# motroy/orion-kmer

Measured on AMD Instinct MI355X. Metric: bases/sec k-mer-counted (k=31) at 1/2/4/8 MI355X; achieved HBM GB/s vs peak, higher is better.
Workload: dtype u64

## Files before the change

orion-kmer_amd/csrc/okm_count.hip:

```cpp
#include "okm_dev_common.h"

namespace okm {

constexpr int kCountWpe = 8;
constexpr int kFullHomeBitsW = 12;

constexpr int kCB = 512;
constexpr int kPer = 8;
constexpr int kCapI = kCB * kPer;
constexpr int kHomeBits = kCB == 512 ? 11 : 10;
constexpr int kHomes = 1 << kHomeBits;
constexpr int kHomesPer = kHomes / kCB;
constexpr int kDenseBits = kHomeBits;
constexpr int kLoadU = 4;

constexpr int kTagBytes = kHomes * 8;
constexpr int kPairBytes = kHomes * 2;
template <bool W> struct Lds {
    static constexpr int kTcntBytes = W ? kHomes * 8 : kPairBytes;
    static constexpr int kRc = kTagBytes + kTcntBytes;
    static constexpr int kHd = kRc + kPairBytes;
    static constexpr int kLt = kHd + kPairBytes;
    static constexpr int kFixed = kLt + kPairBytes;
    static constexpr int kRestEntry = W ? 17 : 9;
// ... 5 lines not shown
    static_assert(kHomes * 12 <= kBytes, "dense mode must fit the carve-up");
};

uint32_t count_item_capacity() { return kCapI; }
uint32_t count_dense_bits() { return kDenseBits; }

template <bool W>
struct CountType {
    typedef uint32_t T;
};
template <>
struct CountType<true> {
    typedef ull T;
};

__device__ __forceinline__ uint32_t wave_incl_scan32(uint32_t v) {
    const int lane = threadIdx.x & 63;
#pragma unroll
    for (int d = 1; d < 64; d <<= 1) {
        const uint32_t o = __shfl_up(v, d, 64);
        if (lane >= d) v += o;
    }
    return v;
}

__device__ __forceinline__ void lds_only_sync();
template <bool LDS_ONLY = false>
__device__ __forceinline__ uint32_t block_excl_scan32(uint32_t v, uint32_t *wsum, uint32_t *total) {
    const int lane = threadIdx.x & 63, wid = threadIdx.x >> 6;
    const uint32_t inc = wave_incl_scan32(v);
    if (lane == 63) wsum[wid] = inc;
    if (LDS_ONLY) lds_only_sync(); else lds_sync();
    uint32_t wbase = 0, tot = 0;
#pragma unroll
    for (int w = 0; w < kCB / 64; ++w) {
        const uint32_t s = wsum[w];
        wbase += w < wid ? s : 0u;
        tot += s;
    }
    if (LDS_ONLY) lds_only_sync(); else lds_sync();
// ... 86 lines not shown
    uint32_t sbase = 0;
    for (uint32_t sg = 0; sg < it.seg_count; ++sg) {
        const DevSeg s = segs[it.seg_begin + sg];
        const uint32_t len = (uint32_t)s.len;
#pragma unroll
        for (int u = 0; u < kPer; ++u) {
            if ((uint32_t)u * kCB >= sbase + len) break;
            const uint32_t f = (uint32_t)u * kCB + t - sbase;
            if (f < len) {
                kk[u] = gload(reinterpret_cast<const KT *>(s.keys) + f);
                if (W && s.counts) ww[u] = gload(s.counts + f);
            }
        }
        sbase += len;
    }
}

constexpr int kSegCache = 64;
template <bool W, typename KT = ull>
__device__ __forceinline__ void load_item_segs(const DevItem &it, const DevSeg *__restrict__ segs, KT (&kk)[kPer],
                                               ull (&ww)[kPer], const uint64_t **ck, const uint64_t **cc,
                                               uint32_t *coff) {
    const uint32_t t = threadIdx.x;
    const uint32_t R = __builtin_amdgcn_readfirstlane(it.seg_count);
    lds_sync();
    if (t < R) {
        const DevSeg s = segs[it.seg_begin + t];
        ck[t] = s.keys;
        cc[t] = s.counts;
        coff[t + 1] = (uint32_t)s.len;
// ... 276 lines not shown
        okeys[p] = sk[b];
        ull c = 0;
        if (W)
            for (uint32_t i = b; i < e; ++i) c += sw[i];
        else
            c = e - b;
        store_count<W>(out_counts, out_off + p, c, narrow, ctl);
    }
    return __builtin_amdgcn_readfirstlane(D);
}


constexpr uint32_t kDeferred = ~0u;

template <bool W, bool NW = false>
__device__ __forceinline__ uint32_t tag_item(const DevItem &it, const DevSeg *__restrict__ segs, uint32_t nrows,
                                             const ull (&kk)[kPer], const ull (&ww)[kPer], ull *lds, uint32_t *wsum,
                                             uint64_t *__restrict__ out_keys, uint64_t *__restrict__ out_counts,
                                             bool narrow, ull *ctl) {
    const uint32_t r = it.rem_bits;
    const uint64_t out_off = it.out_off;
    ull *okeys = out_slot_keys<ull>(it, out_keys);
    typedef Lds<W> L;
    typedef typename CountType<W>::T CT;
    const uint32_t t = threadIdx.x;
    char *base = reinterpret_cast<char *>(lds);
    ull *tag = lds;
    uint32_t *tc16 = reinterpret_cast<uint32_t *>(lds + kHomes);
    ull *tc64 = lds + kHomes;
    uint32_t *rc = reinterpret_cast<uint32_t *>(base + L::kRc);
    uint32_t *hd = reinterpret_cast<uint32_t *>(base + L::kHd);
    uint32_t *lt = reinterpret_cast<uint32_t *>(base + L::kLt);
    ull *rk = reinterpret_cast<ull *>(base + L::kFixed);
    ull *rw = rk + L::kRest;
    uint8_t *rf = reinterpret_cast<uint8_t *>(rk + (W ? 2 : 1) * L::kRest);

    uint32_t hp[kPer];
#pragma unroll
    for (int u = 0; u < kPer; ++u) {
        if ((uint32_t)u >= nrows) break;
        hp[u] = ~0u;
        const ull x = kk[u];
        if (x != kEmptyKey) {
            const uint32_t h = home_of(x, r);
            const ull old = atomicCAS(&tag[h], kEmptyKey, x);
            if (old == kEmptyKey || old == x) {
                if (W)
                    atomicAdd(&tc64[h], ww[u]);
                else
                    atomicAdd(&tc16[h >> 1], 1u << half_shift(h));
            } else {
                const uint32_t o = atomicAdd(&rc[h >> 1], 1u << half_shift(h));
                hp[u] = (h << 16) | half_of(o, h);
            }
        }
    }
    lds_sync();
    hd[2 * t] = hd[2 * t + 1] = 0;
    {
        const uint32_t w0 = rc[2 * t], w1 = rc[2 * t + 1];
        const uint32_t c0 = w0 & 0xFFFFu, c1 = w0 >> 16, c2 = w1 & 0xFFFFu;
        uint32_t rtot;
        const uint32_t a = block_excl_scan32(c0 + c1 + c2 + (w1 >> 16), wsum, &rtot);
// ... 1 lines not shown
            tag_reset<W>(lds);
            return kDeferred;
        }
        rc[2 * t] = a | ((a + c0) << 16);
        rc[2 * t + 1] = (a + c0 + c1) | ((a + c0 + c1 + c2) << 16);
        if (t == 0) wsum[kCB / 64] = rtot;
    }
    lds_sync();
#pragma unroll
    for (int u = 0; u < kPer; ++u) {
        if ((uint32_t)u >= nrows) break;
        if (hp[u] != ~0u) {
            const uint32_t h = hp[u] >> 16;
            const uint32_t dst = half_of(rc[h >> 1], h) + (hp[u] & 0xFFFFu);
            rk[dst] = kk[u];
            if (W) rw[dst] = ww[u];
        }
    }
    lds_sync();
    const uint32_t rtot = __builtin_amdgcn_readfirstlane(wsum[kCB / 64]);
    ull px[L::kRestIters];
    CT pc[L::kRestIters];
    uint32_t prange[L::kRestIters];
#pragma unroll
    for (int k = 0; k < L::kRestIters; ++k) {
        prange[k] = 0;
        if ((uint32_t)k * kCB >= rtot) break;
        const uint32_t p = (uint32_t)k * kCB + t;
        if (p < rtot) {
            const ull x = rk[p];
            const uint32_t h = home_of(x, r);
// ... 44 lines not shown
#pragma unroll
        for (int q = 0; q < kHomesPer; ++q) {
            tg[q] = tag[kHomesPer * t + q];
            tag[kHomesPer * t + q] = kEmptyKey;
            dq[q] += tg[q] != kEmptyKey;
            ho[q] = d;
            d += dq[q];
        }
        const uint32_t od = block_excl_scan32(d, wsum, &D);
#pragma unroll
        for (int q = 0; q < kHomesPer; ++q) ho[q] += od;
        hd[2 * t] = ho[0] | (ho[1] << 16);
        hd[2 * t + 1] = ho[2] | (ho[3] << 16);
    }
    lds_sync();
    {
        const uint32_t lq[kHomesPer] = {lw0 & 0xFFFFu, lw0 >> 16, lw1 & 0xFFFFu, lw1 >> 16};
        uint32_t nq[kHomesPer];
        if (!W) {
            nq[0] = nw0 & 0xFFFFu;
            nq[1] = nw0 >> 16;
            nq[2] = nw1 & 0xFFFFu;
            nq[3] = nw1 >> 16;
        }
#pragma unroll
        for (int q = 0; q < kHomesPer; ++q) {
            if (!NW && tg[q] != kEmptyKey) {
                const uint64_t o = out_off + ho[q] + lq[q];
                okeys[o - out_off] = tg[q];
                const uint64_t cq = W ? (uint64_t)tw[q] : (uint64_t)nq[q];
                store_count<W>(out_counts, o, cq, narrow, ctl);
            }
        }
    }
#pragma unroll
    for (int k = 0; k < L::kRestIters; ++k) {
        if (NW || (uint32_t)k * kCB >= rtot) break;
        if (prange[k]) {
            const ull x = px[k];
            const uint32_t hs = (prange[k] >> 16) & 0x7FFFu, he = prange[k] & 0xFFFFu;
            uint32_t less = 0;
            for (uint32_t q = hs; q < he; ++q) less += (rf[q] && rk[q] < x) ? 1u : 0u;
            const uint32_t h = home_of(x, r);
            const uint32_t tag_below = prange[k] >> 31;
            const uint64_t o = out_off + half_of(hd[h >> 1], h) + less + tag_below;
            okeys[o - out_off] = x;
            store_count<W>(out_counts, o, (uint64_t)pc[k], narrow, ctl);
        }
    }
    return __builtin_amdgcn_readfirstlane(D);
}


template <bool W, typename KT>
__device__ __forceinline__ uint32_t dense_item(const DevItem &it, const DevSeg *__restrict__ segs,
                                               uint64_t *__restrict__ out_keys_raw, uint64_t *__restrict__ out_counts,
                                               ull *lds, uint32_t *wsum, bool nowrite, bool narrow, ull *ctl,
                                               const Direct *dir = nullptr) {
    typedef typename CountType<W>::T CT;
    const uint32_t t = threadIdx.x;
    const uint32_t r = it.rem_bits;
    const uint32_t nslots = 1u << r;
// ... 46 lines not shown
            }
        }
        return __builtin_amdgcn_readfirstlane(D);
    }
    for (uint32_t q = 0; q < kHomesPer; ++q) {
        const uint32_t j = t * kHomesPer + q;
        if (!nowrite && j < nslots && cnt[j] != 0) {
            okeys[o - it.out_off] = slot_key[j];
            store_count<W>(out_counts, o, (uint64_t)cnt[j], narrow, ctl);
            ++o;
        }
    }
    return __builtin_amdgcn_readfirstlane(D);
}

template <bool W, bool NW = false, bool NARROW = !W>
__global__ __launch_bounds__(kCB) __attribute__((amdgpu_waves_per_eu(W ? 1 : kCountWpe)))
void k_count_items(const DevItem *__restrict__ items, uint32_t nitems, const DevSeg *__restrict__ segs,
                   uint64_t *__restrict__ out_keys, uint64_t *__restrict__ out_counts, ull *__restrict__ n_out,
                   ull *__restrict__ ctl, uint32_t *__restrict__ defer, const ull *__restrict__ guard,
                   const ull *__restrict__ d_nitems) {
    if (guard && (guard[0] | guard[1])) return;
    if (d_nitems) nitems = __builtin_amdgcn_readfirstlane((uint32_t)min((ull)nitems, *d_nitems));
    __shared__ __attribute__((aligned(16))) ull lds[Lds<W>::kBytes / 8];
    __shared__ uint32_t wsum[kCB / 64 + 1];
    const uint64_t **seg_k = reinterpret_cast<const uint64_t **>(reinterpret_cast<char *>(lds) + Lds<W>::kFixed);
    const uint64_t **seg_c = seg_k + kSegCache;
    uint32_t *seg_off = reinterpret_cast<uint32_t *>(seg_c + kSegCache);
    static_assert(kSegCache * 20 + 4 <= Lds<W>::kRest * 8, "segment cache fits the rest buffer");
    const uint32_t t = threadIdx.x;
    tag_reset<W>(lds);
    for (uint32_t item = blockIdx.x; item < nitems; item += gridDim.x) {
        const DevItem it = items[item];
        const uint64_t total = it.pad == kItemEmpty ? 0 : item_total(it, segs);
        if (total == 0) {
            if (t == 0) n_out[item] = 0;
            continue;
        }
        uint32_t written = kDeferred;
        if (it.rem_bits > (uint32_t)kDenseBits && total <= (uint64_t)kCapI) {
            ull kk[kPer];
            ull ww[kPer];
            if (W && it.seg_count > 1 && it.seg_count <= (uint32_t)kSegCache)
                load_item_segs<W>(it, segs, kk, ww, seg_k, seg_c, seg_off);
            else
                load_item<W>(it, segs, kk, ww);
            const uint32_t nrows = (uint32_t)((total + kCB - 1) / kCB);
            written = tag_item<W, NW>(it, segs, nrows, kk, ww, lds, wsum, out_keys, out_counts, NARROW, ctl);
        }
        if (t == 0) {
            if (written == kDeferred)
                defer[atomicAdd(reinterpret_cast<unsigned int *>(ctl + 1), 1u)] = item;
            else
                n_out[item] = written;
        }
    }
}

template <typename KT, bool W, bool DIRECT = false>
__global__ __launch_bounds__(kCB) __attribute__((amdgpu_waves_per_eu((W && sizeof(KT) > 8) ? 1 : 4))) void k_count_slow(const DevItem *__restrict__ items, uint32_t nitems,
                                                    const DevSeg *__restrict__ segs,
                                                    uint64_t *__restrict__ out_keys,
                                                    uint64_t *__restrict__ out_counts, ull *__restrict__ n_out,
// ... 52 lines not shown
            written = full_item<W, KT, kHB, DIRECT>(it, (uint32_t)((total + kCB - 1) / kCB), kk, ww, lds, wsum,
                                                    out_keys, out_counts, nowrite, narrow, ctl, dir);
        } else {
            if (threadIdx.x == 0) atomicOr(reinterpret_cast<unsigned int *>(ctl), 2u);
            if (DIRECT) (void)lookback(dsc, 0, ctl);
        }
        if (threadIdx.x == 0) n_out[item] = written;
        lds_sync();
    }
}

void launch_count_items(void *stream, const DevItem *items, uint32_t nitems, const DevSeg *segs,
                        uint64_t *out_keys, uint64_t *out_counts, unsigned long long *n_out,
                        unsigned long long *ctl, uint32_t *defer, bool weighted, bool wide,
                        const unsigned long long *guard, const unsigned long long *d_nitems, bool nowrite,
                        bool narrow) {
    if (!nitems) return;
    hipStream_t s = (hipStream_t)stream;
    constexpr uint32_t wide_cap = 8191, weighted_cap = 4095;
    if (wide) {
        const uint32_t grid = nitems < wide_cap ? nitems : wide_cap;
        if (weighted)
            hipLaunchKernelGGL((k_count_slow<K128, true>), dim3(grid), dim3(kCB), 0, s, items, nitems, segs, out_keys,
                               out_counts, n_out, ctl, (const uint32_t *)nullptr, guard, d_nitems, nowrite, narrow,
                               (ull *)nullptr, (uint64_t *)nullptr, (uint64_t *)nullptr, (const ull *)nullptr);
        else
            hipLaunchKernelGGL((k_count_slow<K128, false>), dim3(grid), dim3(kCB), 0, s, items, nitems, segs,
                               out_keys, out_counts, n_out, ctl, (const uint32_t *)nullptr, guard, d_nitems, nowrite,
                               narrow, (ull *)nullptr, (uint64_t *)nullptr, (uint64_t *)nullptr, (const ull *)nullptr);
        return;
    }
// ... 3 lines not shown
    const uint32_t sgrid = nitems < 1023u ? nitems : 1023u;
    if (weighted) {
        if (nowrite)
            hipLaunchKernelGGL((k_count_items<true, true>), dim3(wgrid), dim3(kCB), 0, s, items, nitems, segs,
                               out_keys, out_counts, n_out, ctl, defer, guard, d_nitems);
        else if (narrow)
            hipLaunchKernelGGL((k_count_items<true, false, true>), dim3(wgrid), dim3(kCB), 0, s, items, nitems, segs,
                               out_keys, out_counts, n_out, ctl, defer, guard, d_nitems);
        else
            hipLaunchKernelGGL((k_count_items<true, false, false>), dim3(wgrid), dim3(kCB), 0, s, items, nitems,
                               segs, out_keys, out_counts, n_out, ctl, defer, guard, d_nitems);
        hipLaunchKernelGGL((k_count_slow<ull, true>), dim3(sgrid), dim3(kCB), 0, s, items, nitems, segs, out_keys,
                           out_counts, n_out, ctl, (const uint32_t *)defer, guard, d_nitems, nowrite, narrow,
                           (ull *)nullptr, (uint64_t *)nullptr, (uint64_t *)nullptr, (const ull *)nullptr);
    } else {
        hipLaunchKernelGGL(k_count_items<false>, dim3(grid), dim3(kCB), 0, s, items, nitems, segs, out_keys,
                           out_counts, n_out, ctl, defer, guard, d_nitems);
        hipLaunchKernelGGL((k_count_slow<ull, false>), dim3(sgrid), dim3(kCB), 0, s, items, nitems, segs, out_keys,
                           out_counts, n_out, ctl, (const uint32_t *)defer, guard, d_nitems, nowrite, narrow,
                           (ull *)nullptr, (uint64_t *)nullptr, (uint64_t *)nullptr, (const ull *)nullptr);
    }
}

void launch_count_direct(void *stream, const DevItem *items, uint32_t nitems, const DevSeg *segs,
                         unsigned long long *n_out, unsigned long long *ctl, bool weighted,
                         const unsigned long long *guard, const unsigned long long *d_nitems,
                         unsigned long long *status, uint64_t *fin_keys, uint64_t *fin_counts,
                         const unsigned long long *fin_base) {
    if (!nitems) return;
    hipStream_t s = (hipStream_t)stream;
    const uint32_t grid = nitems < 2048u ? nitems : 2048u;
    if (weighted)
// ... 11 lines not shown
```

orion-kmer_amd/csrc/okm_dev_common.h:

```cpp
#pragma once

#include <hip/hip_runtime.h>

#include "okm_internal.h"
#include "okm_key.h"

namespace okm {

typedef unsigned long long ull;

__device__ __forceinline__ void lds_sync() { __syncthreads(); }

template <typename T>
__device__ __forceinline__ T gload(const T *p) {
    return *(const __attribute__((address_space(1))) T *)p;
}
__device__ __forceinline__ K128 gload(const K128 *p) {
    typedef unsigned long long u64x2 __attribute__((ext_vector_type(2)));
    const u64x2 v = *(const __attribute__((address_space(1))) u64x2 *)p;
    return K128{v.x, v.y};
}
__device__ __forceinline__ uint4 gload(const uint4 *p) {
    typedef unsigned int u32x4 __attribute__((ext_vector_type(4)));
    const u32x4 v = *(const __attribute__((address_space(1))) u32x4 *)p;
// ... 33 lines not shown
    const int lane = threadIdx.x & 63, wid = threadIdx.x >> 6;
    const ull inc = wave_incl_scan(v);
    if (lane == 63) wsum[wid] = inc;
    lds_sync();
    ull wbase = 0, tot = 0;
#pragma unroll
    for (int w = 0; w < BLOCK / 64; ++w) {
        const ull s = wsum[w];
        if (w < wid) wbase += s;
        tot += s;
    }
    *total = tot;
    return wbase + inc - v;
}

}
```

orion-kmer_amd/csrc/okm_engine.hip:

```cpp
#include <hip/hip_runtime.h>

#include <algorithm>
#include <cmath>
#include <chrono>
#include <cstdio>
#include <cstdlib>
#include <cstring>
#include <map>
#include <memory>
#include <atomic>
#include <mutex>
#include <string>
#include <vector>

#include "okm_arena.h"
#include "okm_hip_try.h"
#include "okm_internal.h"
#include "okm_key.h"
#include "orion_kmer_testing.h"

namespace okm {

static thread_local std::string g_last_error;

// ... 1316 lines not shown
    return OKM_OK;
}

struct ResDst {
    uint64_t *keys, *counts;
    uint64_t off;
    unsigned long long *d_base = nullptr;
    unsigned long long *hslot = nullptr;
};

static okm_status count_and_compact(okm_ctx *c, DevItem *d_items, DevSeg *d_segs, uint32_t nitems,
                                    uint64_t out_total, uint64_t in_total, bool weighted, Blocks &level,
                                    Blocks &items, const unsigned long long *guard = nullptr,
                                    unsigned long long *hguard = nullptr, bool *aborted = nullptr,
                                    const unsigned long long *d_nitems = nullptr, const ResDst *dst = nullptr,
                                    bool last_use = false, bool in_place = false) {
    uint64_t *sk = nullptr, *sc = nullptr;
    unsigned long long *n_out, *dense_off, *scan_tmp;
    const bool direct = dst && c->wide;
    bool narrow = !direct && (!weighted || (!in_place && !dst));
    const uint64_t sc_words = narrow ? (std::max<uint64_t>(out_total, 1) + 1) / 2 : std::max<uint64_t>(out_total, 1);
    if (last_use && c->may_take_runs && !dst && !in_place) {
        const size_t need = std::max<uint64_t>(out_total, 1) * 8 * c->kw;
        size_t best = 0;
        for (auto &r : c->runs) {
            const size_t b = r.borrowed ? 0 : c->pool->size_of(r.keys);
            if (b >= need && (!best || b < best)) best = b, sk = r.keys;
        }
    }
    const bool donated = sk != nullptr;
    Lost lost{c};
// ... 23 lines not shown
                c->pool->size_of(sc) / 1e9, (sk && !donated ? c->pool->size_of(sk) : 0) / 1e9);
    }
    HIP_TRY(hipMemsetAsync(c->flag, 0, 2 * sizeof(unsigned long long), c->stream));
    HIP_TRY(hipMemsetAsync(d_nitems ? n_out : n_out + nitems, 0,
                           (d_nitems ? nitems + 1 : 1) * sizeof(unsigned long long), c->stream));
    if (direct) HIP_TRY(hipMemsetAsync(status, 0, (size_t)nitems * sizeof(unsigned long long), c->stream));
    c->timer.begin(c->stream);
    c->hprof.mark("items.h2d");
    lost.on = donated;
    if (direct)
        launch_count_direct(c->stream, d_items, nitems, d_segs, n_out, c->flag, weighted, guard, d_nitems, status,
                            dst->d_base ? dst->keys : dst->keys + dst->off * c->kw,
                            dst->d_base ? dst->counts : dst->counts + dst->off, dst->d_base);
    else
        launch_count_items(c->stream, d_items, nitems, d_segs, sk, sc, n_out, c->flag, defer, weighted, c->wide, guard,
                           d_nitems, false, narrow);
    c->timer.end(c->stream, "count_items", (8.0 * c->kw + (weighted ? 8.0 : 0.0)) * (double)in_total);
    HIP_TRY(hipGetLastError());
    launch_exclusive_scan(c->stream, n_out, dense_off, nitems + 1, scan_tmp);
    HIP_TRY(hipGetLastError());
    if (dst && !direct) {
        c->timer.begin(c->stream);
        if (dst->d_base)
            launch_compact_items(c->stream, d_items, nitems, n_out, dense_off, sk, sc, dst->keys, dst->counts, c->wide,
                                 !weighted, guard, c->flag, d_nitems, dst->d_base);
        else
            launch_compact_items(c->stream, d_items, nitems, n_out, dense_off, sk, sc, dst->keys + dst->off * c->kw,
                                 dst->counts + dst->off, c->wide, !weighted, guard, c->flag, d_nitems);
        c->timer.end(c->stream, "compact_items", 0.0);
        HIP_TRY(hipGetLastError());
    }
// ... 33 lines not shown
            lost.on = false;
            own.free_all();
            return OKM_OK;
        }
    }
    if (weighted && narrow && hv[1] == 8) {
        c->hprof.mark("count.narrow_overflow");
        own.put(sc);
        sc = nullptr;
        narrow = false;
        OKM_TRY(own.get(std::max<uint64_t>(out_total, 1), &sc));
        HIP_TRY(hipMemsetAsync(c->flag, 0, 2 * sizeof(unsigned long long), c->stream));
        HIP_TRY(hipMemsetAsync(d_nitems ? n_out : n_out + nitems, 0,
                               (d_nitems ? nitems + 1 : 1) * sizeof(unsigned long long), c->stream));
        launch_count_items(c->stream, d_items, nitems, d_segs, sk, sc, n_out, c->flag, defer, weighted, c->wide, guard,
                           d_nitems, false, false);
        HIP_TRY(hipGetLastError());
        launch_exclusive_scan(c->stream, n_out, dense_off, nitems + 1, scan_tmp);
        HIP_TRY(hipMemcpyAsync(&hv[0], dense_off + nitems, sizeof(unsigned long long), hipMemcpyDeviceToHost, c->stream));
        HIP_TRY(hipMemcpyAsync(&hv[1], c->flag, sizeof(unsigned long long), hipMemcpyDeviceToHost, c->stream));
        OKM_TRY(sync(c));
    }
    if (hv[1]) return fail(OKM_E_DEVICE, "count_items invariant violated (code " + std::to_string(hv[1]) + ")");
    const uint64_t nd = hv[0];
    const uint32_t nkept = d_nitems ? (uint32_t)std::min<unsigned long long>(nitems, hv[5]) : nitems;
    const double staged = 8.0 * c->kw + (narrow ? 4.0 : 8.0);
    const double dense = 8.0 * c->kw + 8.0;
    if (!c->timer.stats.empty()) {
        c->timer.stats[c->timer.id_of("count_items")].alg_bytes += (direct ? dense : staged) * (double)nd;
        if (dst && !direct) c->timer.add_bytes("compact_items", (staged + dense) * (double)nd);
    }
// ... 339 lines not shown
                        (unsigned long long)r.n, r.sorted, r.folded, r.borrowed,
                        (unsigned long long)(r.off.empty() ? 0 : r.off.back()));
        }
        bufs.free_all();
        items.free_all();
        *fallback = true;
        return OKM_OK;
    }
    c->info.max_partition = hf[1];
    const int64_t mkv = test_knob(OKM_TEST_SORTED_PATH);
    const double need = 2.0 * (8.0 * c->kw + 8.0) * (double)in_total;
    const bool tight = need > 0.9 * device_room(c);
    const bool two_pass = weighted && (mkv == 2 || (tight && mkv != 1));
    const bool merge = (mkv == 1 || tight) && R <= merge_max_runs() && item_max <= merge_item_capacity();
    if (!two_pass && !merge)
        return count_and_compact(c, d_items, d_segs, nitems, in_total, in_total, weighted, bufs, items);
    items.move_to(bufs);
    if (two_pass) return count_sorted_two_pass(c, d_items, d_segs, nitems, in_total, bufs);
    return merge_sorted_items(c, d_items, d_segs, nitems, in_total, weighted, bufs);
}

struct CountPlan {
    uint32_t twok;
    uint64_t item_max;
    uint32_t capbits;
    uint64_t target;
    uint32_t maxb;
};
static okm_status count_parts(okm_ctx *c, std::vector<DevSeg> &segtab, std::vector<Part> &parts, bool weighted,
                              const CountPlan &cp, const ResDst *dst);
static okm_status count_grouped(okm_ctx *c, std::vector<DevSeg> &segtab, std::vector<Part> &parts, bool weighted,
// ... 427 lines not shown
    }
    c->info.work_items = nitems;
    if (nitems == 0) {
        level.free_all();
        c->counted = true;
        c->n_res = 0;
        c->info.distinct = 0;
        return OKM_OK;
    }
    OKM_TRY(items.get(segtab.size(), &d_segs));
    OKM_TRY(items.get(nitems, &d_items));
    OKM_TRY(h2d(c, d_segs, segtab.data(), segtab.size() * sizeof(DevSeg)));
    OKM_TRY(h2d(c, d_items, host_items.data(), nitems * sizeof(DevItem)));
    c->hprof.mark("items.build");
    return count_and_compact(c, d_items, d_segs, nitems, out_total, in_total, weighted, level, items, nullptr, nullptr,
                             nullptr, nullptr, dst, false, one_seg && !level.held().empty());
}

static okm_status count_grouped(okm_ctx *c, std::vector<DevSeg> &segtab, std::vector<Part> &parts, bool weighted,
                                const CountPlan &cp) {
    uint64_t total = 0;
    for (const Part &p : parts) total += p.len;
    const double ws_key = 8.0 * c->kw * 3 + (weighted ? 8.0 : 4.0) + (weighted ? 16.0 : 0.0);
    const double res_key = 8.0 * c->kw + 8.0;
    const double one_key = std::max(ws_key, 8.0 * c->kw + (weighted ? 8.0 : 4.0) + res_key);
    const double room = device_room(c);
    const double avail = 0.75 * room;
    uint64_t group_keys = total;
    int mode = 0;
    bool over_ok = false;
    if (!weighted && c->may_take_runs && c->runs.size() == 1) {
// ... 823 lines not shown
```

orion-kmer_amd/csrc/okm_extract.hip:

```cpp
#include "okm_scan.h"

namespace okm {

__device__ __forceinline__ uint32_t bin_of(uint64_t key, uint32_t shift) {
    return shift >= 64 ? 0u : (uint32_t)(key >> shift);
}
template <int K>
__device__ __forceinline__ uint32_t bin_k(uint64_t key, uint32_t shift) {
    if (K >= 21) return (uint32_t)(key >> 32) >> (shift - 32u);
    return bin_of(key, shift);
}

constexpr int kExtractBlock = 256;
constexpr int kScatBlock = 1024;
constexpr int kScatWpe = 4;
constexpr int kSegS = 16;
constexpr int kTile = kScatBlock * kSegS;
static_assert(kSegS % 16 == 0, "scan_windows loads whole 16-B words");
constexpr int kSegH = 64;
constexpr int kHTile = kExtractBlock * kSegH;
static_assert(kHTile % kTile == 0, "scatter tile must divide the hist tile");
constexpr int kL1Bits = 9, kL1BitsFold = 10, kL1BitsW = 9;
constexpr int kMaxL1Bins = 1 << kL1BitsFold;
static_assert(2 * 21 - kL1BitsFold >= 32, "bin_k: the L1 shift of k >= 21 lies in the key's high word");
// ... 56 lines not shown
            else
                atomicOr(ovf, 1ull);
        }
        gcur[t] = g;
    }
}

template <int K>
__global__ __launch_bounds__(kScatBlock) __attribute__((amdgpu_waves_per_eu(kScatWpe))) void k_extract_scatter(
    const uint8_t *__restrict__ seq, ExtractGeom g, const uint32_t *__restrict__ HC, ull *__restrict__ cursor,
    uint64_t *__restrict__ out, const ull *__restrict__ cap_end, ull *__restrict__ ovf) {
    __shared__ ull stage[kTile + 64];
    __shared__ ull gcur[kMaxL1Bins];
    __shared__ uint32_t hist[kMaxL1Bins + 1];
    __shared__ uint32_t lofs[kMaxL1Bins];
    __shared__ ull wsum[kScatBlock / 64];
    const uint32_t t = threadIdx.x;
    const uint32_t nb = g.nbins;
    if (t < nb && HC) {
        const uint32_t h = HC[(uint64_t)blockIdx.x * nb + t];
        gcur[t] = h ? atomicAdd(&cursor[t], (ull)h) : 0ull;
    }
    const uint64_t beg = (uint64_t)blockIdx.x * g.chunk;
    const uint64_t end = beg + g.chunk < g.n ? beg + g.chunk : g.n;
    const uint32_t shift = g.shift;
    WinWords<kSegS> ww;
    load_windows_clamped<kSegS>(seq, g.n, beg + (uint64_t)t * kSegS, ww);
    const ull capb = (!HC && t < nb) ? cap_end[t] : 0ull;
    for (uint32_t b = t; b <= nb; b += kScatBlock) hist[b] = 0;
    lds_sync();
    for (uint64_t t0 = beg; t0 < end; t0 += kTile) {
// ... 7 lines not shown
            uint32_t vm = 0;
#pragma unroll
            for (int j = 0; j < kSegS / 2; ++j) rk[j] = 0;
            auto emit = [&](int j, uint64_t key, bool valid) {
                const uint32_t b = valid ? bin_k<K>(key, shift) : nb;
                kk[j] = key;
                rk[j >> 1] |= (atomicAdd(&hist[b], 1u) & 0xFFFFu) << (16 * (j & 1));
                vm |= valid ? 1u << j : 0u;
            };
            if (live) scan_words<kSegS, K>(ww, g.k, emit, g.n - w0);
            load_windows_clamped<kSegS>(seq, g.n, w0 + kTile, ww);
            lds_sync();
            hmine = t <= nb ? hist[t] : 0u;
            if (t <= nb) hist[t] = 0;
            {
                ull tn;
                const uint32_t off = (uint32_t)block_excl_scan_1b<kScatBlock>(t < nb ? hmine : 0u, wsum, &tn);
                if (t < nb) lofs[t] = off;
                tile_n = (uint32_t)tn;
            }
            uint32_t ch = 0;
            ull cp;
            if (!HC && t < nb) {
                ch = hmine;
                cp = atomicAdd(&cursor[t * kL1CurStride], (ull)ch);
            }
            lds_sync();
#pragma unroll
            for (int j = 0; j < kSegS; ++j) {
                const uint32_t rank = (rk[j >> 1] >> (16 * (j & 1))) & 0xFFFFu;
                const uint32_t dst = (vm >> j) & 1u ? lofs[bin_k<K>(kk[j], shift)] + rank : (uint32_t)kTile + (t & 63u);
                stage[dst] = kk[j];
            }
            if (!HC && t < nb) {
// ... 288 lines not shown
```

orion-kmer_amd/csrc/okm_internal.h:

```cpp
#pragma once

#include <stdint.h>
#include <stddef.h>
#include <string>
#include <vector>

#include "orion_kmer.h"

namespace okm {

void set_error(const std::string &msg);
okm_status fail(okm_status s, const std::string &msg);

constexpr uint64_t kEmptyKey = ~0ull;

void *host_pinned_alloc(size_t bytes);
void host_pinned_free(void *p);
okm_status memcpy_d2h_on(int device, void *dst, const void *src, size_t bytes);
int64_t test_knob(int knob);
bool test_fail_alloc();

void trim_device_pools(int device);
void device_bytes_add(int device, int64_t delta);
bool device_over_budget(int device, size_t bytes);
// ... 80 lines not shown
uint32_t extract_max_bins(bool wide);
uint32_t extract_l1_bits(bool wide, bool folding);
uint32_t part_max_bins(bool weighted, bool wide);

size_t scan_tmp_elems(uint64_t n);
void launch_exclusive_scan(void *stream, const unsigned long long *in, unsigned long long *out,
                           uint64_t n, unsigned long long *tmp);

uint32_t count_item_capacity();
uint32_t count_dense_bits();
void launch_count_items(void *stream, const DevItem *items, uint32_t nitems, const DevSeg *segs,
                        uint64_t *out_keys, uint64_t *out_counts, unsigned long long *n_out,
                        unsigned long long *ctl, uint32_t *defer, bool weighted, bool wide,
                        const unsigned long long *guard = nullptr, const unsigned long long *d_nitems = nullptr,
                        bool nowrite = false,
                        bool narrow = false);
void launch_count_direct(void *stream, const DevItem *items, uint32_t nitems, const DevSeg *segs,
                         unsigned long long *n_out, unsigned long long *ctl, bool weighted,
                         const unsigned long long *guard, const unsigned long long *d_nitems,
                         unsigned long long *status, uint64_t *fin_keys, uint64_t *fin_counts,
                         const unsigned long long *fin_base);

uint32_t merge_item_capacity();
uint32_t merge_max_runs();
void launch_merge_items(void *stream, const DevItem *items, uint32_t nitems, const DevSeg *segs,
                        unsigned long long *n_out, const unsigned long long *dense_off, uint64_t *out_keys,
                        uint64_t *out_counts, unsigned long long *ctl, bool weighted, bool wide, bool write);

struct DevParent {
    uint32_t out_base;
    uint32_t rem;
// ... 67 lines not shown
```

orion-kmer_amd/csrc/okm_partition.hip:

```cpp
#include "okm_dev_common.h"

namespace okm {

constexpr int kPartBlock = 1024;
constexpr int kHistU = 4;

uint32_t part_max_bins(bool weighted, bool wide) {
    return weighted ? 512u : (!wide ? 2u * kPartBlock : (uint32_t)kPartBlock);
}

template <typename KT>
__device__ __forceinline__ uint32_t local_bin(const KT &key, const DevSeg &s) {
    const uint64_t b = (s.shift >= (uint32_t)KeyOps<KT>::kBits ? 0ull : KeyOps<KT>::shr(key, s.shift)) - s.key_base;
    return b < s.nlocal ? (uint32_t)b : s.nlocal - 1;
}

template <typename KT>
__device__ __forceinline__ void hist_key(const KT &key, const DevSeg &s, uint32_t *lh) {
    if (!KeyOps<KT>::is_empty(key)) atomicAdd(&lh[local_bin(key, s)], 1u);
}

template <typename KT>
__global__ __launch_bounds__(kPartBlock) void k_part_hist(const DevSeg *__restrict__ segs,
                                                          const DevChunk *__restrict__ chunks,
// ... 56 lines not shown
template <typename KT, bool W, bool BIG = false>
__global__ __launch_bounds__(kPartBlock) __attribute__((amdgpu_waves_per_eu(1)))
void k_part_scatter_tile(
    const DevSeg *__restrict__ segs, const DevChunk *__restrict__ chunks, uint32_t nchunks,
    uint32_t max_local, const uint32_t *__restrict__ HC, ull *__restrict__ cursor,
    uint64_t *__restrict__ out_keys_raw, uint64_t *__restrict__ out_counts, const ull *__restrict__ cap_end,
    ull *__restrict__ ovf) {
    constexpr int T = Tile<KT, W, BIG>::kKeys, P = Tile<KT, W, BIG>::kPer;
    constexpr uint32_t BPT = BIG ? 2 : 1;
    extern __shared__ __attribute__((aligned(16))) ull lds[];
    KT *stage = reinterpret_cast<KT *>(lds);
    ull *cstage = reinterpret_cast<ull *>(stage + T);
    ull *gcur = W ? cstage + T : cstage;
    uint32_t *hist = reinterpret_cast<uint32_t *>(gcur + max_local);
    uint32_t *lofs = hist + max_local;
    __shared__ ull wsum[kPartBlock / 64];
    KT *out_keys = reinterpret_cast<KT *>(out_keys_raw);
    const uint32_t t = threadIdx.x;

    for (uint32_t c = blockIdx.x; c < nchunks; c += gridDim.x) {
        const DevChunk ch = chunks[c];
        const DevSeg s = segs[ch.seg];
        const uint32_t nl = s.nlocal;
        if (HC)
            for (uint32_t b = t; b < nl; b += kPartBlock) {
                const uint32_t h = HC[(uint64_t)c * max_local + b];
                gcur[b] = h ? atomicAdd(&cursor[s.out_base + b], (ull)h) : 0ull;
            }
        const KT *keys = reinterpret_cast<const KT *>(s.keys) + ch.begin;
        const uint64_t *cnts = s.counts ? s.counts + ch.begin : nullptr;
        for (uint64_t base = 0; base < ch.len; base += T) {
// ... 19 lines not shown
            lds_sync();
            uint32_t my[BPT];
            uint32_t mine = 0;
#pragma unroll
            for (uint32_t q = 0; q < BPT; ++q) {
                const uint32_t b = BPT * t + q;
                my[q] = b < nl ? hist[b] : 0u;
                mine += my[q];
            }
            ull claim[BPT];
#pragma unroll
            for (uint32_t q = 0; q < BPT; ++q) {
                claim[q] = 0;
                if (!HC && my[q]) claim[q] = atomicAdd(&cursor[s.out_base + BPT * t + q], (ull)my[q]);
            }
            ull tile_n;
            uint32_t off = (uint32_t)block_excl_scan<kPartBlock>(mine, wsum, &tile_n);
#pragma unroll
            for (uint32_t q = 0; q < BPT; ++q) {
                if (BPT * t + q < nl) lofs[BPT * t + q] = off;
                off += my[q];
            }
            lds_sync();
#pragma unroll
            for (int u = 0; u < P; ++u) {
                if (br[u] != ~0u) {
                    const uint32_t dst = lofs[br[u] >> 16] + (br[u] & 0xFFFFu);
                    stage[dst] = kk[u];
                    if (W) cstage[dst] = ww[u];
                }
            }
            if (!HC) {
#pragma unroll
                for (uint32_t q = 0; q < BPT; ++q) {
                    const uint32_t b = BPT * t + q;
                    if (b >= nl) continue;
                    ull g = ~0ull;
                    if (my[q]) {
                        if (claim[q] + my[q] <= cap_end[s.out_base + b])
                            g = claim[q];
                        else
                            atomicOr(ovf, 1ull);
                    }
                    gcur[b] = g;
                }
            }
            lds_sync();
            for (uint32_t j = t; j < (uint32_t)tile_n; j += kPartBlock) {
                const KT key = stage[j];
                const uint32_t b = local_bin(key, s);
                const ull g = gcur[b];
                if (g == ~0ull) continue;
                const ull o = g + (j - lofs[b]);
                out_keys[o] = key;
                if (W) out_counts[o] = cstage[j];
            }
            lds_sync();
            if (HC)
                for (uint32_t b = t; b < nl; b += kPartBlock) gcur[b] += hist[b];
        }
        lds_sync();
    }
}
// ... 70 lines not shown
```

Measured before the change: 113.3 billion.

## Add single-segment count kernel, DPP wave scan, and 32-bit block scans

Adds a specialized unweighted count-items kernel for the single-segment case. It loads keys directly from keys0 without the segment loop and reads item fields through a pointer instead of copying the whole struct. The shuffle-based wave scan is replaced with DPP row operations. Partition and extract now use a 32-bit block scan in place of the 64-bit one, and output stores go through address-space-1 pointer arithmetic with 32-bit indices. These changes aim to cut instruction count, register use and cross-lane overhead, at the cost of another template variant and new correctness assumptions, such as indices fitting in 32 bits and the item layout.

After: 121.7 billion, median of 6. 1.07x the previous value.

```diff
diff --git a/orion-kmer_amd/csrc/okm_count.hip b/orion-kmer_amd/csrc/okm_count.hip
--- a/orion-kmer_amd/csrc/okm_count.hip
+++ b/orion-kmer_amd/csrc/okm_count.hip
@@ -43,16 +43,6 @@
     typedef ull T;
 };
 
-__device__ __forceinline__ uint32_t wave_incl_scan32(uint32_t v) {
-    const int lane = threadIdx.x & 63;
-#pragma unroll
-    for (int d = 1; d < 64; d <<= 1) {
-        const uint32_t o = __shfl_up(v, d, 64);
-        if (lane >= d) v += o;
-    }
-    return v;
-}
-
 __device__ __forceinline__ void lds_only_sync();
 template <bool LDS_ONLY = false>
 __device__ __forceinline__ uint32_t block_excl_scan32(uint32_t v, uint32_t *wsum, uint32_t *total) {
@@ -169,6 +159,22 @@
         }
         sbase += len;
     }
+}
+
+__device__ __forceinline__ void load_item_one(const uint64_t *__restrict__ keys, uint32_t len, ull (&kk)[kPer]) {
+    const uint32_t t = threadIdx.x;
+#pragma unroll
+    for (int u = 0; u < kPer; ++u) {
+        const uint32_t f = (uint32_t)u * kCB + t;
+        kk[u] = kEmptyKey;
+        if (f < len) kk[u] = gload(reinterpret_cast<const ull *>(keys) + f);
+    }
+}
+
+typedef __attribute__((address_space(1))) char gchar;
+template <typename T>
+__device__ __forceinline__ void gstore_at(gchar *base, uint32_t idx, T v) {
+    *reinterpret_cast<__attribute__((address_space(1))) T *>(base + idx * (uint32_t)sizeof(T)) = v;
 }
 
 constexpr int kSegCache = 64;
@@ -475,13 +481,10 @@
 constexpr uint32_t kDeferred = ~0u;
 
 template <bool W, bool NW = false>
-__device__ __forceinline__ uint32_t tag_item(const DevItem &it, const DevSeg *__restrict__ segs, uint32_t nrows,
-                                             const ull (&kk)[kPer], const ull (&ww)[kPer], ull *lds, uint32_t *wsum,
-                                             uint64_t *__restrict__ out_keys, uint64_t *__restrict__ out_counts,
-                                             bool narrow, ull *ctl) {
-    const uint32_t r = it.rem_bits;
-    const uint64_t out_off = it.out_off;
-    ull *okeys = out_slot_keys<ull>(it, out_keys);
+__device__ __forceinline__ uint32_t tag_item(const DevItem *__restrict__ ip, uint32_t r, uint32_t nrows,
+                                             const ull (&kk)[kPer], const ull (&ww)[W ? kPer : 1], ull *lds,
+                                             uint32_t *wsum, uint64_t *__restrict__ out_keys,
+                                             uint64_t *__restrict__ out_counts, bool narrow, ull *ctl) {
     typedef Lds<W> L;
     typedef typename CountType<W>::T CT;
     const uint32_t t = threadIdx.x;
@@ -498,16 +501,17 @@
 
     uint32_t hp[kPer];
 #pragma unroll
+    for (int u = 0; u < kPer; ++u) hp[u] = ~0u;
+#pragma unroll
     for (int u = 0; u < kPer; ++u) {
         if ((uint32_t)u >= nrows) break;
-        hp[u] = ~0u;
         const ull x = kk[u];
         if (x != kEmptyKey) {
             const uint32_t h = home_of(x, r);
             const ull old = atomicCAS(&tag[h], kEmptyKey, x);
             if (old == kEmptyKey || old == x) {
                 if (W)
-                    atomicAdd(&tc64[h], ww[u]);
+                    atomicAdd(&tc64[h], ww[W ? u : 0]);
                 else
                     atomicAdd(&tc16[h >> 1], 1u << half_shift(h));
             } else {
@@ -539,7 +543,7 @@
             const uint32_t h = hp[u] >> 16;
             const uint32_t dst = half_of(rc[h >> 1], h) + (hp[u] & 0xFFFFu);
             rk[dst] = kk[u];
-            if (W) rw[dst] = ww[u];
+            if (W) rw[dst] = ww[W ? u : 0];
         }
     }
     lds_sync();
@@ -614,6 +618,20 @@
         hd[2 * t + 1] = ho[2] | (ho[3] << 16);
     }
     lds_sync();
+    if (NW) return __builtin_amdgcn_readfirstlane(D);
+    const uint64_t out_off = ip->out_off;
+    gchar *const okeys = out_keys ? (gchar *)(out_keys + out_off) : (gchar *)ip->keys0;
+    const bool c64 = W && !narrow;
+    gchar *const ocnt = (gchar *)out_counts + out_off * (c64 ? 8u : 4u);
+    auto put = [&](uint32_t o, ull key, uint64_t c) {
+        gstore_at<ull>(okeys, o, key);
+        if (c64) {
+            gstore_at<ull>(ocnt, o, c);
+        } else {
+            if (W && c > 0xFFFFFFFFull) atomicOr(reinterpret_cast<unsigned int *>(ctl), 8u);
+            gstore_at<uint32_t>(ocnt, o, (uint32_t)c);
+        }
+    };
     {
         const uint32_t lq[kHomesPer] = {lw0 & 0xFFFFu, lw0 >> 16, lw1 & 0xFFFFu, lw1 >> 16};
         uint32_t nq[kHomesPer];
@@ -625,17 +643,12 @@
         }
 #pragma unroll
         for (int q = 0; q < kHomesPer; ++q) {
-            if (!NW && tg[q] != kEmptyKey) {
-                const uint64_t o = out_off + ho[q] + lq[q];
-                okeys[o - out_off] = tg[q];
-                const uint64_t cq = W ? (uint64_t)tw[q] : (uint64_t)nq[q];
-                store_count<W>(out_counts, o, cq, narrow, ctl);
-            }
+            if (tg[q] != kEmptyKey) put(ho[q] + lq[q], tg[q], W ? (uint64_t)tw[W ? q : 0] : (uint64_t)nq[q]);
         }
     }
 #pragma unroll
     for (int k = 0; k < L::kRestIters; ++k) {
-        if (NW || (uint32_t)k * kCB >= rtot) break;
+        if ((uint32_t)k * kCB >= rtot) break;
         if (prange[k]) {
             const ull x = px[k];
             const uint32_t hs = (prange[k] >> 16) & 0x7FFFu, he = prange[k] & 0xFFFFu;
@@ -643,9 +656,7 @@
             for (uint32_t q = hs; q < he; ++q) less += (rf[q] && rk[q] < x) ? 1u : 0u;
             const uint32_t h = home_of(x, r);
             const uint32_t tag_below = prange[k] >> 31;
-            const uint64_t o = out_off + half_of(hd[h >> 1], h) + less + tag_below;
-            okeys[o - out_off] = x;
-            store_count<W>(out_counts, o, (uint64_t)pc[k], narrow, ctl);
+            put(half_of(hd[h >> 1], h) + less + tag_below, x, (uint64_t)pc[k]);
         }
     }
     return __builtin_amdgcn_readfirstlane(D);
@@ -722,7 +733,7 @@
     return __builtin_amdgcn_readfirstlane(D);
 }
 
-template <bool W, bool NW = false, bool NARROW = !W>
+template <bool W, bool NW = false, bool NARROW = !W, bool SEG1 = false>
 __global__ __launch_bounds__(kCB) __attribute__((amdgpu_waves_per_eu(W ? 1 : kCountWpe)))
 void k_count_items(const DevItem *__restrict__ items, uint32_t nitems, const DevSeg *__restrict__ segs,
                    uint64_t *__restrict__ out_keys, uint64_t *__restrict__ out_counts, ull *__restrict__ n_out,
@@ -738,8 +749,34 @@
     static_assert(kSegCache * 20 + 4 <= Lds<W>::kRest * 8, "segment cache fits the rest buffer");
     const uint32_t t = threadIdx.x;
     tag_reset<W>(lds);
+    static_assert(!(SEG1 && W), "the single-segment kernel is the unweighted one");
     for (uint32_t item = blockIdx.x; item < nitems; item += gridDim.x) {
-        const DevItem it = items[item];
+        const DevItem *ip = items + item;
+        if (SEG1) {
+            const uint64_t total = ip->pad == kItemEmpty ? 0 : ip->total;
+            if (total == 0) {
+                if (t == 0) n_out[item] = 0;
+                continue;
+            }
+            uint32_t written = kDeferred;
+            const uint32_t r = ip->rem_bits;
+            if (r > (uint32_t)kDenseBits && total <= (uint64_t)kCapI && ip->seg_count == 1) {
+                const uint32_t len = (uint32_t)total;
+                const uint32_t nrows = (len + kCB - 1) / kCB;
+                ull kk[kPer];
+                const ull none[1] = {1};
+                load_item_one(ip->keys0, len, kk);
+                written = tag_item<false, NW>(ip, r, nrows, kk, none, lds, wsum, out_keys, out_counts, NARROW, ctl);
+            }
+            if (t == 0) {
+                if (written == kDeferred)
+                    defer[atomicAdd(reinterpret_cast<unsigned int *>(ctl + 1), 1u)] = item;
+                else
+                    n_out[item] = written;
+            }
+            continue;
+        }
+        const DevItem it = *ip;
         const uint64_t total = it.pad == kItemEmpty ? 0 : item_total(it, segs);
         if (total == 0) {
             if (t == 0) n_out[item] = 0;
@@ -754,7 +791,12 @@
             else
                 load_item<W>(it, segs, kk, ww);
             const uint32_t nrows = (uint32_t)((total + kCB - 1) / kCB);
-            written = tag_item<W, NW>(it, segs, nrows, kk, ww, lds, wsum, out_keys, out_counts, NARROW, ctl);
+            if constexpr (W) {
+                written = tag_item<W, NW>(ip, it.rem_bits, nrows, kk, ww, lds, wsum, out_keys, out_counts, NARROW, ctl);
+            } else {
+                const ull none[1] = {1};
+                written = tag_item<W, NW>(ip, it.rem_bits, nrows, kk, none, lds, wsum, out_keys, out_counts, NARROW, ctl);
+            }
         }
         if (t == 0) {
             if (written == kDeferred)
@@ -837,7 +879,7 @@
                         uint64_t *out_keys, uint64_t *out_counts, unsigned long long *n_out,
                         unsigned long long *ctl, uint32_t *defer, bool weighted, bool wide,
                         const unsigned long long *guard, const unsigned long long *d_nitems, bool nowrite,
-                        bool narrow) {
+                        bool narrow, bool multi_seg) {
     if (!nitems) return;
     hipStream_t s = (hipStream_t)stream;
     constexpr uint32_t wide_cap = 8191, weighted_cap = 4095;
@@ -871,8 +913,12 @@
                            out_counts, n_out, ctl, (const uint32_t *)defer, guard, d_nitems, nowrite, narrow,
                            (ull *)nullptr, (uint64_t *)nullptr, (uint64_t *)nullptr, (const ull *)nullptr);
     } else {
-        hipLaunchKernelGGL(k_count_items<false>, dim3(grid), dim3(kCB), 0, s, items, nitems, segs, out_keys,
-                           out_counts, n_out, ctl, defer, guard, d_nitems);
+        if (multi_seg)
+            hipLaunchKernelGGL(k_count_items<false>, dim3(grid), dim3(kCB), 0, s, items, nitems, segs, out_keys,
+                               out_counts, n_out, ctl, defer, guard, d_nitems);
+        else
+            hipLaunchKernelGGL((k_count_items<false, false, true, true>), dim3(grid), dim3(kCB), 0, s, items, nitems,
+                               segs, out_keys, out_counts, n_out, ctl, defer, guard, d_nitems);
         hipLaunchKernelGGL((k_count_slow<ull, false>), dim3(sgrid), dim3(kCB), 0, s, items, nitems, segs, out_keys,
                            out_counts, n_out, ctl, (const uint32_t *)defer, guard, d_nitems, nowrite, narrow,
                            (ull *)nullptr, (uint64_t *)nullptr, (uint64_t *)nullptr, (const ull *)nullptr);
diff --git a/orion-kmer_amd/csrc/okm_dev_common.h b/orion-kmer_amd/csrc/okm_dev_common.h
--- a/orion-kmer_amd/csrc/okm_dev_common.h
+++ b/orion-kmer_amd/csrc/okm_dev_common.h
@@ -71,4 +71,32 @@
     return wbase + inc - v;
 }
 
+__device__ __forceinline__ uint32_t wave_incl_scan32(uint32_t v) {
+    v += (uint32_t)__builtin_amdgcn_update_dpp(0, (int)v, 0x111, 0xF, 0xF, false);
+    v += (uint32_t)__builtin_amdgcn_update_dpp(0, (int)v, 0x112, 0xF, 0xF, false);
+    v += (uint32_t)__builtin_amdgcn_update_dpp(0, (int)v, 0x114, 0xF, 0xF, false);
+    v += (uint32_t)__builtin_amdgcn_update_dpp(0, (int)v, 0x118, 0xF, 0xF, false);
+    v += (uint32_t)__builtin_amdgcn_update_dpp(0, (int)v, 0x142, 0xA, 0xF, false);
+    v += (uint32_t)__builtin_amdgcn_update_dpp(0, (int)v, 0x143, 0xC, 0xF, false);
+    return v;
 }
+
+template <int BLOCK, bool TRAILING = true>
+__device__ __forceinline__ uint32_t block_excl_scan_u32(uint32_t v, uint32_t *wsum, uint32_t *total) {
+    const int lane = threadIdx.x & 63, wid = threadIdx.x >> 6;
+    const uint32_t inc = wave_incl_scan32(v);
+    if (lane == 63) wsum[wid] = inc;
+    lds_sync();
+    uint32_t wbase = 0, tot = 0;
+#pragma unroll
+    for (int w = 0; w < BLOCK / 64; ++w) {
+        const uint32_t s = wsum[w];
+        wbase += w < wid ? s : 0u;
+        tot += s;
+    }
+    if (TRAILING) lds_sync();
+    *total = tot;
+    return wbase + inc - v;
+}
+
+}
diff --git a/orion-kmer_amd/csrc/okm_engine.hip b/orion-kmer_amd/csrc/okm_engine.hip
--- a/orion-kmer_amd/csrc/okm_engine.hip
+++ b/orion-kmer_amd/csrc/okm_engine.hip
@@ -1354,7 +1354,7 @@
                                     Blocks &items, const unsigned long long *guard = nullptr,
                                     unsigned long long *hguard = nullptr, bool *aborted = nullptr,
                                     const unsigned long long *d_nitems = nullptr, const ResDst *dst = nullptr,
-                                    bool last_use = false, bool in_place = false) {
+                                    bool last_use = false, bool in_place = false, bool multi_seg = false) {
     uint64_t *sk = nullptr, *sc = nullptr;
     unsigned long long *n_out, *dense_off, *scan_tmp;
     const bool direct = dst && c->wide;
@@ -1408,7 +1408,7 @@
                             dst->d_base ? dst->counts : dst->counts + dst->off, dst->d_base);
     else
         launch_count_items(c->stream, d_items, nitems, d_segs, sk, sc, n_out, c->flag, defer, weighted, c->wide, guard,
-                           d_nitems, false, narrow);
+                           d_nitems, false, narrow, multi_seg);
     c->timer.end(c->stream, "count_items", (8.0 * c->kw + (weighted ? 8.0 : 0.0)) * (double)in_total);
     HIP_TRY(hipGetLastError());
     launch_exclusive_scan(c->stream, n_out, dense_off, nitems + 1, scan_tmp);
@@ -1472,7 +1472,7 @@
         HIP_TRY(hipMemsetAsync(d_nitems ? n_out : n_out + nitems, 0,
                                (d_nitems ? nitems + 1 : 1) * sizeof(unsigned long long), c->stream));
         launch_count_items(c->stream, d_items, nitems, d_segs, sk, sc, n_out, c->flag, defer, weighted, c->wide, guard,
-                           d_nitems, false, false);
+                           d_nitems, false, false, multi_seg);
         HIP_TRY(hipGetLastError());
         launch_exclusive_scan(c->stream, n_out, dense_off, nitems + 1, scan_tmp);
         HIP_TRY(hipMemcpyAsync(&hv[0], dense_off + nitems, sizeof(unsigned long long), hipMemcpyDeviceToHost, c->stream));
@@ -1842,7 +1842,8 @@
     const bool two_pass = weighted && (mkv == 2 || (tight && mkv != 1));
     const bool merge = (mkv == 1 || tight) && R <= merge_max_runs() && item_max <= merge_item_capacity();
     if (!two_pass && !merge)
-        return count_and_compact(c, d_items, d_segs, nitems, in_total, in_total, weighted, bufs, items);
+        return count_and_compact(c, d_items, d_segs, nitems, in_total, in_total, weighted, bufs, items, nullptr, nullptr,
+                                 nullptr, nullptr, nullptr, false, false, true);
     items.move_to(bufs);
     if (two_pass) return count_sorted_two_pass(c, d_items, d_segs, nitems, in_total, bufs);
     return merge_sorted_items(c, d_items, d_segs, nitems, in_total, weighted, bufs);
@@ -2300,7 +2301,7 @@
     OKM_TRY(h2d(c, d_items, host_items.data(), nitems * sizeof(DevItem)));
     c->hprof.mark("items.build");
     return count_and_compact(c, d_items, d_segs, nitems, out_total, in_total, weighted, level, items, nullptr, nullptr,
-                             nullptr, nullptr, dst, false, one_seg && !level.held().empty());
+                             nullptr, nullptr, dst, false, one_seg && !level.held().empty(), !one_seg);
 }
 
 static okm_status count_grouped(okm_ctx *c, std::vector<DevSeg> &segtab, std::vector<Part> &parts, bool weighted,
diff --git a/orion-kmer_amd/csrc/okm_extract.hip b/orion-kmer_amd/csrc/okm_extract.hip
--- a/orion-kmer_amd/csrc/okm_extract.hip
+++ b/orion-kmer_amd/csrc/okm_extract.hip
@@ -94,7 +94,7 @@
     __shared__ ull gcur[kMaxL1Bins];
     __shared__ uint32_t hist[kMaxL1Bins + 1];
     __shared__ uint32_t lofs[kMaxL1Bins];
-    __shared__ ull wsum[kScatBlock / 64];
+    __shared__ uint32_t wsum[kScatBlock / 64];
     const uint32_t t = threadIdx.x;
     const uint32_t nb = g.nbins;
     if (t < nb && HC) {
@@ -132,10 +132,8 @@
             hmine = t <= nb ? hist[t] : 0u;
             if (t <= nb) hist[t] = 0;
             {
-                ull tn;
-                const uint32_t off = (uint32_t)block_excl_scan_1b<kScatBlock>(t < nb ? hmine : 0u, wsum, &tn);
+                const uint32_t off = block_excl_scan_u32<kScatBlock, false>(t < nb ? hmine : 0u, wsum, &tile_n);
                 if (t < nb) lofs[t] = off;
-                tile_n = (uint32_t)tn;
             }
             uint32_t ch = 0;
             ull cp;
diff --git a/orion-kmer_amd/csrc/okm_internal.h b/orion-kmer_amd/csrc/okm_internal.h
--- a/orion-kmer_amd/csrc/okm_internal.h
+++ b/orion-kmer_amd/csrc/okm_internal.h
@@ -118,7 +118,8 @@
                         unsigned long long *ctl, uint32_t *defer, bool weighted, bool wide,
                         const unsigned long long *guard = nullptr, const unsigned long long *d_nitems = nullptr,
                         bool nowrite = false,
-                        bool narrow = false);
+                        bool narrow = false,
+                        bool multi_seg = false);
 void launch_count_direct(void *stream, const DevItem *items, uint32_t nitems, const DevSeg *segs,
                          unsigned long long *n_out, unsigned long long *ctl, bool weighted,
                          const unsigned long long *guard, const unsigned long long *d_nitems,
diff --git a/orion-kmer_amd/csrc/okm_partition.hip b/orion-kmer_amd/csrc/okm_partition.hip
--- a/orion-kmer_amd/csrc/okm_partition.hip
+++ b/orion-kmer_amd/csrc/okm_partition.hip
@@ -94,7 +94,7 @@
     ull *gcur = W ? cstage + T : cstage;
     uint32_t *hist = reinterpret_cast<uint32_t *>(gcur + max_local);
     uint32_t *lofs = hist + max_local;
-    __shared__ ull wsum[kPartBlock / 64];
+    __shared__ uint32_t wsum[kPartBlock / 64];
     KT *out_keys = reinterpret_cast<KT *>(out_keys_raw);
     const uint32_t t = threadIdx.x;
 
@@ -144,8 +144,8 @@
                 claim[q] = 0;
                 if (!HC && my[q]) claim[q] = atomicAdd(&cursor[s.out_base + BPT * t + q], (ull)my[q]);
             }
-            ull tile_n;
-            uint32_t off = (uint32_t)block_excl_scan<kPartBlock>(mine, wsum, &tile_n);
+            uint32_t tile_n;
+            uint32_t off = block_excl_scan_u32<kPartBlock>(mine, wsum, &tile_n);
 #pragma unroll
             for (uint32_t q = 0; q < BPT; ++q) {
                 if (BPT * t + q < nl) lofs[BPT * t + q] = off;
@@ -176,7 +176,7 @@
                 }
             }
             lds_sync();
-            for (uint32_t j = t; j < (uint32_t)tile_n; j += kPartBlock) {
+            for (uint32_t j = t; j < tile_n; j += kPartBlock) {
                 const KT key = stage[j];
                 const uint32_t b = local_bin(key, s);
                 const ull g = gcur[b];
```
